# EleutherAI/DALLE-mtf

Measured on AMD Instinct MI355X. Metric: train tokens/sec (text+image) per node, dalle_example, higher is better.
Workload: dtype bf16

## Files before the change

### dalle-mtf_amd/csrc/gemm.hip

```cpp
#include "common.h"
#include <string.h>
#include <type_traits>

static int g_opt_nt4 = 1;
static int g_opt_nt8 = 1;
int g_opt_reserve_cus = 0;
int g_opt_attn_fwd = 1;
int g_opt_attn_bwd = 1;
int g_opt_attn_xcd = 8;
static int g_opt_tn8 = 0;
static int g_opt_tn8_max_tiles = 16;
static int g_opt_nt8_min_k = 2048;
static int g_opt_skinny = 1;
static int g_opt_tn_wide = 1;
static int g_opt_tn_tail = 1;
static int g_opt_cstream = 1;
static int g_opt_cstream_min_mb = 256;
static int g_opt_cstream_nt_min_mb = 1024;
static int g_opt_res16 = 1;
static int g_opt_ntr = 1;
static int g_opt_nt8p = 1;
static int g_opt_relu_bits = 1;
static int g_opt_nt8p_max_k = 1024;
static int g_opt_nt4_lds = 49152;
unsigned long long* g_dbg_buf = nullptr;
extern "C" int dmi_set_debug_buffer(void* p) { g_dbg_buf = (unsigned long long*)p; return 0; }
extern "C" int dmi_get_option(const char* name) {
  if (!strcmp(name, "nt4")) return g_opt_nt4;
  if (!strcmp(name, "nt8")) return g_opt_nt8;
  if (!strcmp(name, "tn_tail")) return g_opt_tn_tail;
  if (!strcmp(name, "tn_wide")) return g_opt_tn_wide;
  if (!strcmp(name, "nt4_lds")) return g_opt_nt4_lds;
  if (!strcmp(name, "nt8p")) return g_opt_nt8p;
  if (!strcmp(name, "ntr")) return g_opt_ntr;
  if (!strcmp(name, "cstream")) return g_opt_cstream;
  if (!strcmp(name, "cstream_min_mb")) return g_opt_cstream_min_mb;
  if (!strcmp(name, "cstream_nt_min_mb")) return g_opt_cstream_nt_min_mb;
  if (!strcmp(name, "nt8p_max_k")) return g_opt_nt8p_max_k;
  if (!strcmp(name, "relu_bits")) return g_opt_relu_bits;
  if (!strcmp(name, "res16")) return g_opt_res16;
  if (!strcmp(name, "skinny")) return g_opt_skinny;
  if (!strcmp(name, "nt8_min_k")) return g_opt_nt8_min_k;
  if (!strcmp(name, "tn8")) return g_opt_tn8;
  if (!strcmp(name, "tn8_max_tiles")) return g_opt_tn8_max_tiles;
  if (!strcmp(name, "attn_xcd")) return g_opt_attn_xcd;
  if (!strcmp(name, "attn_fwd")) return g_opt_attn_fwd;
  if (!strcmp(name, "attn_bwd")) return g_opt_attn_bwd;
  if (!strcmp(name, "reserve_cus")) return g_opt_reserve_cus;
  return -1;
}
extern "C" int dmi_set_option(const char* name, int value) {
  if (!strcmp(name, "nt4")) { g_opt_nt4 = value; return 0; }
  if (!strcmp(name, "nt8")) { g_opt_nt8 = value; return 0; }
  if (!strcmp(name, "tn_tail")) { g_opt_tn_tail = value; return 0; }
  if (!strcmp(name, "tn_wide")) { g_opt_tn_wide = value; return 0; }
  if (!strcmp(name, "nt4_lds")) { if (value < 49152 || value > 163840) return -1; g_opt_nt4_lds = value; return 0; }
  if (!strcmp(name, "nt8p")) { g_opt_nt8p = value; return 0; }
  if (!strcmp(name, "ntr")) { g_opt_ntr = value; return 0; }
  if (!strcmp(name, "cstream")) { g_opt_cstream = value; return 0; }
  if (!strcmp(name, "cstream_min_mb")) { g_opt_cstream_min_mb = value; return 0; }
  if (!strcmp(name, "cstream_nt_min_mb")) { g_opt_cstream_nt_min_mb = value; return 0; }
  if (!strcmp(name, "nt8p_max_k")) { g_opt_nt8p_max_k = value; return 0; }
  if (!strcmp(name, "relu_bits")) { g_opt_relu_bits = value; return 0; }
  if (!strcmp(name, "res16")) { g_opt_res16 = value; return 0; }
  if (!strcmp(name, "skinny")) { g_opt_skinny = value; return 0; }
  if (!strcmp(name, "nt8_min_k")) { g_opt_nt8_min_k = value; return 0; }
  if (!strcmp(name, "tn8")) { g_opt_tn8 = value; return 0; }
  if (!strcmp(name, "tn8_max_tiles")) { g_opt_tn8_max_tiles = value; return 0; }
  if (!strcmp(name, "attn_xcd")) { g_opt_attn_xcd = value; return 0; }
  if (!strcmp(name, "attn_fwd")) { g_opt_attn_fwd = value; return 0; }
  if (!strcmp(name, "attn_bwd")) { g_opt_attn_bwd = value; return 0; }
  if (!strcmp(name, "reserve_cus")) { if (value < 0) return -1; g_opt_reserve_cus = value; return 0; }
  return -1;
}

#define BM 128
#define BN 128
#define BK 64
#ifndef GROUP_M
#define GROUP_M 8
#endif

struct GemmArgs {
  const bf16_t* A;
  const bf16_t* B;
  void* C;
  const bf16_t* bias;
  const bf16_t* residual;
  const bf16_t* relu_src;
  unsigned short* relu_bits;
  const float* rowscale;
// ... 888 lines not shown
      const u32x2 graw = *(const u32x2*)(a.ln_gamma + n), braw = *(const u32x2*)(a.ln_beta + n);
      const float g0 = __uint_as_float(graw[0] << 16), g1 = __uint_as_float(graw[0] & 0xffff0000u);
      const float g2 = __uint_as_float(graw[1] << 16), g3 = __uint_as_float(graw[1] & 0xffff0000u);
      const float b0 = __uint_as_float(braw[0] << 16), b1 = __uint_as_float(braw[0] & 0xffff0000u);
      const float b2 = __uint_as_float(braw[1] << 16), b3 = __uint_as_float(braw[1] & 0xffff0000u);
#pragma unroll
      for (int t = 0; t < RT; ++t) {
        P[t][jj][0] = pack2bf(acc[t][j][0] * rs[t] * g0 + b0, acc[t][j][1] * rs[t] * g1 + b1);
        P[t][jj][1] = pack2bf(acc[t][j][2] * rs[t] * g2 + b2, acc[t][j][3] * rs[t] * g3 + b3);
      }
    }
#pragma unroll
    for (int t = 0; t < RT; ++t) {
      const int m = m0 + wm * (RM / 2) + 16 * t + c16;
#pragma unroll
      for (int d = 0; d < 2; ++d) { swap16(P[t][0][d], P[t][1][d]); swap16(P[t][2][d], P[t][3][d]); }
      if (m < a.M) {
        bf16_t* yp = a.ln_y + (int64_t)m * a.ln_ldy + ncolw + 64 * h + pcol;
        *(u32x4*)yp = u32x4{P[t][0][0], P[t][0][1], P[t][1][0], P[t][1][1]};
        *(u32x4*)(yp + 32) = u32x4{P[t][2][0], P[t][2][1], P[t][3][0], P[t][3][1]};
      }
    }
  }
}

__device__ __forceinline__ float dpp_row_sum16(float v) {
  v += __builtin_bit_cast(float, __builtin_amdgcn_update_dpp(0, __builtin_bit_cast(int, v), 0xB1, 0xf, 0xf, false));
  v += __builtin_bit_cast(float, __builtin_amdgcn_update_dpp(0, __builtin_bit_cast(int, v), 0x4E, 0xf, 0xf, false));
  v += __builtin_bit_cast(float, __builtin_amdgcn_update_dpp(0, __builtin_bit_cast(int, v), 0x141, 0xf, 0xf, false));
  v += __builtin_bit_cast(float, __builtin_amdgcn_update_dpp(0, __builtin_bit_cast(int, v), 0x140, 0xf, 0xf, false));
  return v;
}
template <int RT>
__device__ __forceinline__ void epilogue_lnbwd(const GemmArgs& a, f32x4 (&acc)[RT][8], char* smem, int lane, int wm, int wn, int m0) {
  constexpr int RM = 32 * RT;
  const int c16 = lane & 15, g16 = lane >> 4;
  float* red = (float*)smem;
  const int ncolw = wn * 128;
  const int pcol = 8 * (((g16 & 1) << 1) | (g16 >> 1));
  const float invn = 1.0f / 512.0f;
  const int nbytes = (int)(((int64_t)(a.M - m0) * 512) * 2);
  const __amdgpu_buffer_rsrc_t rx = __builtin_amdgcn_make_buffer_rsrc((void*)(a.ln_x + (int64_t)m0 * 512), 0, nbytes, 0x00020000);
  const __amdgpu_buffer_rsrc_t rr = __builtin_amdgcn_make_buffer_rsrc((void*)((a.residual ? a.residual : a.ln_x) + (int64_t)m0 * 512), 0,
                                                                       a.residual ? nbytes : 0, 0x00020000);
  const __amdgpu_buffer_rsrc_t ry = __builtin_amdgcn_make_buffer_rsrc((void*)(a.ln_y + (int64_t)m0 * 512), 0, nbytes, 0x00020000);
  const __amdgpu_buffer_rsrc_t rmu = __builtin_amdgcn_make_buffer_rsrc((void*)(a.ln_mean + m0), 0, (a.M - m0) * 4, 0x00020000);
  const __amdgpu_buffer_rsrc_t rrs = __builtin_amdgcn_make_buffer_rsrc((void*)(a.ln_rstd + m0), 0, (a.M - m0) * 4, 0x00020000);
  const int r0 = wm * (RM / 2) + c16;
  float* prow = a.ln_part + (int64_t)(blockIdx.x * 2 + wm) * 1024;
  auto lo = [](unsigned w) { return __uint_as_float(w << 16); };
  auto hi = [](unsigned w) { return __uint_as_float(w & 0xffff0000u); };
  unsigned dyp[RT][8][2], xp[RT][8][2];
  const int vst = (r0 * 512 + ncolw + pcol) * 2;
  auto ld16 = [&](const __amdgpu_buffer_rsrc_t rsrc, int voff, int imm) {
    return __builtin_bit_cast(u32x4, __builtin_amdgcn_raw_buffer_load_b128(rsrc, voff, imm, 0));
  };
  auto ldmu = [&](int t) { return __builtin_bit_cast(float, __builtin_amdgcn_raw_buffer_load_b32(rmu, r0 * 4 + 64 * t, 0, 0)); };
  auto ldrs = [&](int t) { return __builtin_bit_cast(float, __builtin_amdgcn_raw_buffer_load_b32(rrs, r0 * 4 + 64 * t, 0, 0)); };
  const bf16_t* gp = a.ln_gamma + ncolw + 4 * g16;
#pragma unroll
  for (int t = 0; t < RT; ++t)
#pragma unroll
    for (int h = 0; h < 2; ++h) {
      const u32x4 l0 = ld16(rx, vst + 16384 * t + 128 * h, 0), l1 = ld16(rx, vst + 16384 * t + 128 * h + 64, 0);
      xp[t][4 * h + 0][0] = l0[0]; xp[t][4 * h + 0][1] = l0[1]; xp[t][4 * h + 1][0] = l0[2]; xp[t][4 * h + 1][1] = l0[3];
      xp[t][4 * h + 2][0] = l1[0]; xp[t][4 * h + 2][1] = l1[1]; xp[t][4 * h + 3][0] = l1[2]; xp[t][4 * h + 3][1] = l1[3];
    }
#pragma unroll
  for (int t = 0; t < RT; ++t)
#pragma unroll
    for (int j = 0; j < 8; ++j) {
      dyp[t][j][0] = pack2bf(acc[t][j][0], acc[t][j][1]); dyp[t][j][1] = pack2bf(acc[t][j][2], acc[t][j][3]);
      asm volatile("" : "+v"(dyp[t][j][0]), "+v"(dyp[t][j][1]));
    }
#pragma unroll
  for (int t = 0; t < RT; ++t)
#pragma unroll
    for (int h = 0; h < 2; ++h)
#pragma unroll
      for (int dd = 0; dd < 2; ++dd) { swap16(xp[t][4 * h][dd], xp[t][4 * h + 1][dd]); swap16(xp[t][4 * h + 2][dd], xp[t][4 * h + 3][dd]); }
  auto opaque = [&]() {
#pragma unroll
    for (int t = 0; t < RT; ++t)
#pragma unroll
      for (int j = 0; j < 8; ++j) asm volatile("" : "+v"(dyp[t][j][0]), "+v"(dyp[t][j][1]), "+v"(xp[t][j][0]), "+v"(xp[t][j][1]));
  };
  opaque();
  float s1[RT], s2[RT];
  {
    unsigned gmp[8][2];
#pragma unroll
    for (int j = 0; j < 8; ++j) {
      const u32x2 graw = *(const u32x2*)(gp + 16 * j);
      gmp[j][0] = graw[0]; gmp[j][1] = graw[1];
    }
#pragma unroll
    for (int t = 0; t < RT; ++t) {
      const float mu = ldmu(t), rs = ldrs(t);
      float a1 = 0.f, a2 = 0.f;
#pragma unroll
      for (int j = 0; j < 8; ++j) {
        const float xv[4] = {lo(xp[t][j][0]), hi(xp[t][j][0]), lo(xp[t][j][1]), hi(xp[t][j][1])};
        const float dy[4] = {lo(dyp[t][j][0]), hi(dyp[t][j][0]), lo(dyp[t][j][1]), hi(dyp[t][j][1])};
        const float gm[4] = {lo(gmp[j][0]), hi(gmp[j][0]), lo(gmp[j][1]), hi(gmp[j][1])};
#pragma unroll
        for (int e = 0; e < 4; ++e) {
          const float xh = (xv[e] - mu) * rs;
          const float gy = dy[e] * gm[e];
          a1 += gy;
          a2 += gy * xh;
        }
      }
      s1[t] = a1; s2[t] = a2;
      __builtin_amdgcn_sched_barrier(0);
    }
  }
#pragma unroll
  for (int t = 0; t < RT; ++t) {
    s1[t] += __shfl_xor(s1[t], 16, 64); s1[t] += __shfl_xor(s1[t], 32, 64);
    s2[t] += __shfl_xor(s2[t], 16, 64); s2[t] += __shfl_xor(s2[t], 32, 64);
    if (g16 == 0) {
      float* q = red + ((r0 + 16 * t) * 4 + wn) * 2;
      q[0] = s1[t]; q[1] = s2[t];
    }
  }
  __syncthreads();
  opaque();
  {
    float mu[RT], rs[RT];
#pragma unroll
    for (int t = 0; t < RT; ++t) { mu[t] = ldmu(t); rs[t] = ldrs(t); }
#pragma unroll
    for (int j = 0; j < 8; ++j) {
      float ag[4] = {0.f, 0.f, 0.f, 0.f}, ab[4] = {0.f, 0.f, 0.f, 0.f};
#pragma unroll
      for (int t = 0; t < RT; ++t) {
        const float xv[4] = {lo(xp[t][j][0]), hi(xp[t][j][0]), lo(xp[t][j][1]), hi(xp[t][j][1])};
        const float dy[4] = {lo(dyp[t][j][0]), hi(dyp[t][j][0]), lo(dyp[t][j][1]), hi(dyp[t][j][1])};
#pragma unroll
        for (int e = 0; e < 4; ++e) {
          ab[e] += dy[e];
          ag[e] += dy[e] * ((xv[e] - mu[t]) * rs[t]);
        }
      }
      f32x4 pg, pb;
#pragma unroll
      for (int e = 0; e < 4; ++e) { pg[e] = dpp_row_sum16(ag[e]); pb[e] = dpp_row_sum16(ab[e]); }
      if (c16 == 0) {
        const int n = ncolw + 16 * j + 4 * g16;
        *(f32x4*)(prow + n) = pg;
        *(f32x4*)(prow + 512 + n) = pb;
      }
      __builtin_amdgcn_sched_barrier(0);
    }
  }
  opaque();
#pragma unroll
  for (int t = 0; t < RT; ++t) {
    const f32x4 q0 = *(const f32x4*)(red + (r0 + 16 * t) * 8);
    const f32x4 q1 = *(const f32x4*)(red + (r0 + 16 * t) * 8 + 4);
    const float m1 = ((q0[0] + q0[2]) + (q1[0] + q1[2])) * invn;
    const float m2 = ((q0[1] + q0[3]) + (q1[1] + q1[3])) * invn;
    const float mu = ldmu(t), rs = ldrs(t);
#pragma unroll
    for (int h = 0; h < 2; ++h) {
      const u32x4 l0 = ld16(rr, vst + 16384 * t + 128 * h, 0), l1 = ld16(rr, vst + 16384 * t + 128 * h + 64, 0);
      unsigned R[4][2] = {{l0[0], l0[1]}, {l0[2], l0[3]}, {l1[0], l1[1]}, {l1[2], l1[3]}};
#pragma unroll
      for (int dd = 0; dd < 2; ++dd) { swap16(R[0][dd], R[1][dd]); swap16(R[2][dd], R[3][dd]); }
      unsigned P[4][2];
#pragma unroll
      for (int jj = 0; jj < 4; ++jj) {
        const int j = 4 * h + jj;
        const u32x2 graw = *(const u32x2*)(gp + 16 * j);
        const float xv[4] = {lo(xp[t][j][0]), hi(xp[t][j][0]), lo(xp[t][j][1]), hi(xp[t][j][1])};
        const float rv[4] = {lo(R[jj][0]), hi(R[jj][0]), lo(R[jj][1]), hi(R[jj][1])};
        const float gm[4] = {lo(graw[0]), hi(graw[0]), lo(graw[1]), hi(graw[1])};
        const float dy[4] = {lo(dyp[t][j][0]), hi(dyp[t][j][0]), lo(dyp[t][j][1]), hi(dyp[t][j][1])};
        float o[4];
#pragma unroll
        for (int e = 0; e < 4; ++e) {
          const float xh = (xv[e] - mu) * rs;
          o[e] = rs * (dy[e] * gm[e] - m1 - xh * m2) + rv[e];
        }
        P[jj][0] = pack2bf(o[0], o[1]);
        P[jj][1] = pack2bf(o[2], o[3]);
      }
#pragma unroll
      for (int dd = 0; dd < 2; ++dd) { swap16(P[0][dd], P[1][dd]); swap16(P[2][dd], P[3][dd]); }
      __builtin_amdgcn_raw_buffer_store_b128(u32x4{P[0][0], P[0][1], P[1][0], P[1][1]}, ry, vst + 16384 * t + 128 * h, 0, 0);
      __builtin_amdgcn_raw_buffer_store_b128(u32x4{P[2][0], P[2][1], P[3][0], P[3][1]}, ry, vst + 16384 * t + 128 * h + 64, 0, 0);
      __builtin_amdgcn_sched_barrier(0);
    }
  }
}

template <int FLAGS, int RT, int LN = 0>
__global__ __launch_bounds__(512, 2) void gemm_ntr_kernel(GemmArgs a) {
  extern __shared__ __attribute__((aligned(16))) char smem[];
  constexpr int RM = 32 * RT;
  constexpr int ABYTES = RM * 64;
  constexpr int BUF = ABYTES + 32768;
  constexpr int NPA = RM / 16;
  constexpr int NP = NPA + 32;
  constexpr int PW = (NP + 7) / 8;
  const int tid = threadIdx.x, lane = tid & 63;
  const int wid = __builtin_amdgcn_readfirstlane(tid >> 6);
  const int wm = wid >> 2, wn = wid & 3;
  const int m0 = blockIdx.x * RM;
  int ns = a.K / 32;

  const int c16 = lane & 15, g16 = lane >> 4;
  int offa = lds4_off(wm * (RM / 2) + c16, g16);
  int offb = ABYTES + lds4_off(wn * 128 + c16, g16);
  __amdgpu_buffer_rsrc_t ra = __builtin_amdgcn_make_buffer_rsrc((void*)(a.A + (int64_t)m0 * a.lda), 0,
                                                                 (int)(((int64_t)(a.M - 1 - m0) * a.lda + a.K) * 2), 0x00020000);
  __amdgpu_buffer_rsrc_t rb = __builtin_amdgcn_make_buffer_rsrc((void*)a.B, 0, (int)(((int64_t)(a.N - 1) * a.ldb + a.K) * 2), 0x00020000);
  int vo[PW];
  auto set_offsets = [&](int lda_, int ldb_, int ln) {
#pragma unroll
    for (int q = 0; q < PW; ++q) {
      const int p = wid + 8 * q;
      const bool isa = p < NPA;
      const int row = 16 * (isa ? p : p - NPA) + (ln >> 2), pc = ln & 3;
      vo[q] = (row * (isa ? lda_ : ldb_) + 8 * (pc ^ lds4_swz(row))) * 2;
    }
  };
  set_offsets(a.lda, a.ldb, lane);
  auto piece = [&](int buf, int q, int soff) {
    const int p = wid + 8 * q;
    if (p >= NP) return;
    char* dst = smem + buf * BUF + (p < NPA ? p * 1024 : ABYTES + (p - NPA) * 1024);
    if (p < NPA) glds16(ra, dst, vo[q], soff);
    else glds16(rb, dst, vo[q], soff);
  };

  f32x4 acc[RT][8];
#pragma unroll
  for (int i = 0; i < RT; ++i)
#pragma unroll
    for (int j = 0; j < 8; ++j) acc[i][j] = f32x4{0.f, 0.f, 0.f, 0.f};

  auto compute = [&](int buf, int nbuf, int soff) {
    const char* cur = smem + buf * BUF;
    bf16x8 fb[8], fa[RT];
#pragma unroll
    for (int j = 0; j < 8; ++j) fb[j] = *(const bf16x8*)(cur + offb + j * 1024);
    fa[0] = *(const bf16x8*)(cur + offa);
    if (RT > 1) fa[1] = *(const bf16x8*)(cur + offa + 1024);
    MFMA_PRIO(1);
#pragma unroll
    for (int i = 0; i < RT; ++i) {
      if (i + 2 < RT) fa[i + 2] = *(const bf16x8*)(cur + offa + (i + 2) * 1024);
#pragma unroll
      for (int j = 0; j < 8; ++j)
        acc[i][j] = __builtin_amdgcn_mfma_f32_16x16x32_bf16(fb[j], fa[i], acc[i][j], 0, 0, 0);
#pragma unroll
      for (int q = 2 * i; q < 2 * i + 2; ++q)
        if (q < PW) piece(nbuf, q, soff);
      __builtin_amdgcn_sched_barrier(0);
    }
    MFMA_PRIO(0);
  };

  auto mainloop = [&]() {
#pragma unroll
    for (int q = 0; q < PW; ++q) piece(0, q, 0);
#pragma unroll
    for (int q = 0; q < PW; ++q) piece(1, q, ns > 1 ? 64 : 0);
    asm volatile("s_waitcnt vmcnt(0)" ::: "memory");
    __syncthreads();
    for (int s = 0; s < ns; s += 3) {
#pragma unroll
      for (int u = 0; u < 3; ++u) {
        if (s + u < ns) {
          const int q = s + u + 2;
          compute(u, (u + 2) % 3, (q < ns ? q : 0) * 64);
          asm volatile("s_waitcnt vmcnt(%0)" ::"n"(PW - 1) : "memory");
          __builtin_amdgcn_s_barrier();
        }
      }
    }
    asm volatile("s_waitcnt vmcnt(0)" ::: "memory");
  };
  mainloop();
  if constexpr (LN == 3) {
    __syncthreads();
    {
      int lane_e = (int)__builtin_amdgcn_mbcnt_hi(~0u, __builtin_amdgcn_mbcnt_lo(~0u, 0u));
      asm volatile("" : "+v"(lane_e));
      epilogue_lnbwd<RT>(a, acc, smem, lane_e, wm, wn, m0);
    }
    asm volatile("s_waitcnt vmcnt(0)" ::: "memory");
    __syncthreads();
    ra = __builtin_amdgcn_make_buffer_rsrc((void*)(a.ln_y + (int64_t)m0 * a.ln_ldy), 0, (int)(((int64_t)(a.M - 1 - m0) * a.ln_ldy + a.N) * 2), 0x00020000);
    rb = __builtin_amdgcn_make_buffer_rsrc((void*)a.B2, 0, (int)(((int64_t)(a.N - 1) * a.ldb2 + a.N) * 2), 0x00020000);
    int lane2 = (int)__builtin_amdgcn_mbcnt_hi(~0u, __builtin_amdgcn_mbcnt_lo(~0u, 0u));
    asm volatile("" : "+v"(lane2));
    offa = lds4_off(wm * (RM / 2) + (lane2 & 15), lane2 >> 4);
    offb = ABYTES + lds4_off(wn * 128 + (lane2 & 15), lane2 >> 4);
    set_offsets(a.ln_ldy, a.ldb2, lane2);
    ns = a.N / 32;
#pragma unroll
    for (int i = 0; i < RT; ++i)
#pragma unroll
      for (int j = 0; j < 8; ++j) acc[i][j] = f32x4{0.f, 0.f, 0.f, 0.f};
    mainloop();
    GemmArgs b2 = a;
    b2.C = a.C2; b2.ldc = a.N; b2.cpol = 0;
    f32x4 lo[RT][4], hi[RT][4];
#pragma unroll
    for (int i = 0; i < RT; ++i)
#pragma unroll
      for (int j = 0; j < 4; ++j) { lo[i][j] = acc[i][j]; hi[i][j] = acc[i][j + 4]; }
    epilogue_regs<0, RT>(b2, lo, lane2, m0 + wm * (RM / 2), wn * 128);
    epilogue_regs<0, RT>(b2, hi, lane2, m0 + wm * (RM / 2), wn * 128 + 64);
  } else if constexpr (LN != 0) {
    __syncthreads();
    if constexpr (LN == 1) epilogue_ln<RT>(a, acc, smem, lane, wm, wn, m0);
    else {
      int lane_e = lane;
      asm volatile("" : "+v"(lane_e));
      epilogue_lnbwd<RT>(a, acc, smem, lane_e, wm, wn, m0);
    }
  } else {
    f32x4 lo[RT][4], hi[RT][4];
#pragma unroll
    for (int i = 0; i < RT; ++i)
#pragma unroll
      for (int j = 0; j < 4; ++j) { lo[i][j] = acc[i][j]; hi[i][j] = acc[i][j + 4]; }
    epilogue_regs<FLAGS, RT>(a, lo, lane, m0 + wm * (RM / 2), wn * 128);
    epilogue_regs<FLAGS, RT>(a, hi, lane, m0 + wm * (RM / 2), wn * 128 + 64);
  }
}

__global__ __launch_bounds__(256) void reduce_slabs_kernel(const float* __restrict__ slabs, float* __restrict__ out,
                                                           int nsplit, int64_t n4, int64_t stride4) {
  for (int64_t i = (int64_t)blockIdx.x * 256 + threadIdx.x; i < n4; i += (int64_t)gridDim.x * 256) {
    f32x4 acc = ((const f32x4*)slabs)[i];
    for (int s = 1; s < nsplit; ++s) {
      const f32x4 v = ((const f32x4*)slabs)[s * stride4 + i];
      acc[0] += v[0]; acc[1] += v[1]; acc[2] += v[2]; acc[3] += v[3];
    }
    ((f32x4*)out)[i] = acc;
  }
}

#define SK_WAVES 8
template <int FLAGS>
__global__ __launch_bounds__(64 * SK_WAVES) void gemm_nt_skinny_kernel(const GemmArgs a) {
  __shared__ f32x4 red[SK_WAVES][2][64];
  const int lane = threadIdx.x & 63, wid = threadIdx.x >> 6;
  const int c = lane & 15, g = lane >> 4;
  const int n0 = blockIdx.x * 16;
  const int r0 = c < a.M ? c : a.M - 1, r1 = 16 + c < a.M ? 16 + c : a.M - 1;
  const bf16_t* pa0 = a.A + (int64_t)r0 * a.lda + 16 * g;
// ... 136 lines not shown
static int num_cus() {
  static int n = 0;
  if (!n) {
    int dev = 0;
    hipDeviceProp_t prop;
    if (hipGetDevice(&dev) == hipSuccess && hipGetDeviceProperties(&prop, dev) == hipSuccess) n = prop.multiProcessorCount;
    if (n < 8) n = 256;
  }
  return n;
}

static int persistent_grid() {
  int n = (num_cus() - g_opt_reserve_cus) & ~7;
  return n < 8 ? 8 : n;
}

static bool nt8p_can(const GemmArgs& a) {
  return a.k_per_split == a.K && a.K % 128 == 0 && (int64_t)a.M * a.lda < (1 << 30) && (int64_t)a.N * a.ldb < (1 << 30);
}
static bool nt8p_auto(int M, int N, int K) {
  return K <= g_opt_nt8p_max_k && ((M + BM8 - 1) / BM8) * ((N + BN8 - 1) / BN8) >= 2 * num_cus();
}
template <int FLAGS>
static int launch_nt8p(const GemmArgs& a, hipStream_t st) {
  static bool attr8p = false;
  if (!attr8p) { (void)hipFuncSetAttribute((const void*)gemm_nt8p_kernel<FLAGS>, hipFuncAttributeMaxDynamicSharedMemorySize, 131072); attr8p = true; }
  GemmArgs b = a;
  b.tiles_m = (a.M + BM8 - 1) / BM8; b.tiles_n = (a.N + BN8 - 1) / BN8;
  gemm_nt8p_kernel<FLAGS><<<dim3(persistent_grid()), dim3(512), 131072, st>>>(b);
  DMI_CHECK_LAUNCH("gemm_nt8p");
  return DMI_OK;
}

template <int FLAGS>
static int launch_nt(const GemmArgs& a, int nsplit, hipStream_t st) {
  const dim3 grid(a.tiles_m * a.tiles_n, nsplit), blk(256);
  if constexpr (FLAGS == 0 || FLAGS == DMI_GEMM_BIAS || FLAGS == (DMI_GEMM_BIAS | DMI_GEMM_RELU) || FLAGS == (DMI_GEMM_BIAS | DMI_GEMM_RESIDUAL)) {
    if (g_opt_skinny && a.M <= 32 && nsplit == 1 && a.N % 16 == 0) {
      gemm_nt_skinny_kernel<FLAGS><<<dim3(a.N / 16), dim3(64 * SK_WAVES), 0, st>>>(a);
      DMI_CHECK_LAUNCH("gemm_nt_skinny");
      return DMI_OK;
    }
  }
  if constexpr (epi_regs_ok<FLAGS> && !(FLAGS & GEMM_SOFTMAX)) {
    if (g_opt_ntr && a.N == 512 && nsplit == 1 && a.k_per_split == a.K && a.K % 32 == 0 && (int64_t)a.N * a.ldb < (1 << 30) &&
        (g_opt_ntr == 2 || (a.M >= 160 * (num_cus() / 2) && a.K <= 4096 && g_opt_reserve_cus == 0))) {
      constexpr int RT = 5;
      constexpr int LDSB = 3 * (32 * RT * 64 + 32768);
      static bool attrr = false;
      if (!attrr) { (void)hipFuncSetAttribute((const void*)gemm_ntr_kernel<FLAGS, RT>, hipFuncAttributeMaxDynamicSharedMemorySize, LDSB); attrr = true; }
      GemmArgs b = a;
      b.pf = g_opt_res16 ? 2 : 0;
      gemm_ntr_kernel<FLAGS, RT><<<dim3((a.M + 32 * RT - 1) / (32 * RT)), dim3(512), LDSB, st>>>(b);
      DMI_CHECK_LAUNCH("gemm_ntr");
      return DMI_OK;
    }
  }
  if constexpr (epi_regs_ok<FLAGS>) {
    const bool can = nsplit == 1 && nt8p_can(a);
    const bool auto_ok = nt8p_auto(a.M, a.N, a.K);
    if (can && ((g_opt_nt8p == 1 && auto_ok) || g_opt_nt8p == 2 || (g_opt_nt8p == 3 && (FLAGS & GEMM_SOFTMAX) && auto_ok)))
      return launch_nt8p<FLAGS>(a, st);
  }
  {
    const int t8m = (a.M + BM8 - 1) / BM8, t8n = (a.N + BN8 - 1) / BN8;
    const bool auto8 = g_opt_nt8 == 1 && a.k_per_split >= g_opt_nt8_min_k && (t8m * t8n * nsplit) % 256 == 0;
    if (auto8 || g_opt_nt8 == 2) {
      static bool attr8 = false;
      if (!attr8) { (void)hipFuncSetAttribute((const void*)gemm_nt8_kernel<FLAGS>, hipFuncAttributeMaxDynamicSharedMemorySize, 131072); attr8 = true; }
      GemmArgs b = a;
      b.tiles_m = t8m; b.tiles_n = t8n;
      gemm_nt8_kernel<FLAGS><<<dim3(t8m * t8n, nsplit), dim3(512), 131072, st>>>(b);
      DMI_CHECK_LAUNCH("gemm_nt8");
      return DMI_OK;
    }
  }
  if constexpr (!(FLAGS & DMI_GEMM_OUT_F32)) {
    const int tiles4 = ((a.M + BM4 - 1) / BM4) * a.tiles_n;
    if (g_opt_nt4 && nsplit == 1 && a.k_per_split == a.K && ((tiles4 >= 1536 && a.K <= 1024) || g_opt_nt4 == 2)) {
      static int attr4 = 0;
      if (attr4 != g_opt_nt4_lds) { (void)hipFuncSetAttribute((const void*)gemm_nt4_kernel<FLAGS>, hipFuncAttributeMaxDynamicSharedMemorySize, g_opt_nt4_lds); attr4 = g_opt_nt4_lds; }
      GemmArgs b = a;
      b.tiles_m = (a.M + BM4 - 1) / BM4;
      gemm_nt4_kernel<FLAGS><<<dim3(tiles4), blk, g_opt_nt4_lds, st>>>(b);
      DMI_CHECK_LAUNCH("gemm_nt4");
      return DMI_OK;
// ... 83 lines not shown
extern "C" int dmi_gemm_nt_mask_bits(const uint16_t* A, int lda, const uint16_t* Bt, int ldb, uint16_t* C, int ldc, int M, int N, int K,
                                     const void* bits, void* stream) {
  int rc = check_nt(A, lda, Bt, ldb, C, ldc, M, N, K);
  if (rc) return rc;
  GemmArgs a;
  fill_nt_args(a, A, lda, Bt, ldb, C, ldc, M, N, K);
  a.relu_bits = (unsigned short*)bits; a.dbg = g_dbg_buf;
  if ((rc = check_bits("gemm_nt_mask_bits", a, bits))) return rc;
  return launch_nt8p<GEMM_MASK_BITS>(a, (hipStream_t)stream);
}

extern "C" int dmi_gemm_nt_ln_auto(int M, int N, int K) {
  if (M <= 0 || N != 512 || K <= 0 || K % BK != 0) return 0;
  if ((int64_t)N * K >= (1 << 30) || (int64_t)M * K >= ((int64_t)1 << 31) || (int64_t)M * N * 2 >= ((int64_t)1 << 31)) return 0;
  return g_opt_reserve_cus == 0 ? 1 : 0;
}

extern "C" int dmi_gemm_nt_ln(const uint16_t* A, int lda, const uint16_t* Bt, int ldb, uint16_t* C, int ldc, int M, int N, int K,
                              const uint16_t* bias, const uint16_t* residual, const uint16_t* gamma, const uint16_t* beta, float eps,
                              uint16_t* Y, int ldy, float* mean, float* rstd, void* stream) {
  int rc = check_nt(A, lda, Bt, ldb, C, ldc, M, N, K);
  if (rc) return rc;
  DMI_REQUIRE(gamma && beta && Y && mean && rstd, "gemm_nt_ln: null pointer");
  DMI_REQUIRE((((uintptr_t)gamma | (uintptr_t)beta | (uintptr_t)Y | (uintptr_t)bias | (uintptr_t)residual) & 15) == 0 && ldy % 8 == 0 && ldy >= N,
              "gemm_nt_ln: operands must be 16-byte aligned");
  if (N != 512 || (int64_t)N * ldb >= (1 << 30) || (int64_t)M * lda >= ((int64_t)1 << 31)) {
    dmi_set_error("gemm_nt_ln: the fused form needs N = 512 (one block owns whole rows); got N=%d", N);
    return DMI_ERR_UNSUPPORTED;
  }
  GemmArgs a;
  fill_nt_args(a, A, lda, Bt, ldb, C, ldc, M, N, K);
  a.bias = bias; a.residual = residual;
  a.ln_gamma = gamma; a.ln_beta = beta; a.ln_y = Y; a.ln_ldy = ldy; a.ln_mean = mean; a.ln_rstd = rstd; a.ln_eps = eps;
  constexpr int RT = 5;
  constexpr int LDSB = 3 * (32 * RT * 64 + 32768);
  static bool attr = false;
  if (!attr) { (void)hipFuncSetAttribute((const void*)gemm_ntr_kernel<0, RT, 1>, hipFuncAttributeMaxDynamicSharedMemorySize, LDSB); attr = true; }
  gemm_ntr_kernel<0, RT, 1><<<dim3((M + 32 * RT - 1) / (32 * RT)), dim3(512), LDSB, (hipStream_t)stream>>>(a);
  DMI_CHECK_LAUNCH("gemm_nt_ln");
  return DMI_OK;
}

extern "C" int dmi_gemm_nt_lnbwd_parts(int M) { return 2 * ((M + 159) / 160); }
extern "C" int dmi_gemm_nt_lnbwd(const uint16_t* A, int lda, const uint16_t* Bt, int ldb, int M, int N, int K, const uint16_t* x,
                                 const uint16_t* gamma, const float* mean, const float* rstd, const uint16_t* dres, uint16_t* dx,
                                 float* part, const uint16_t* B2, int ldb2, uint16_t* C2, void* stream) {
  int rc = check_nt(A, lda, Bt, ldb, dx, N, M, N, K);
  if (rc) return rc;
  DMI_REQUIRE(x && gamma && mean && rstd && part, "gemm_nt_lnbwd: null pointer");
  DMI_REQUIRE((((uintptr_t)x | (uintptr_t)gamma | (uintptr_t)dres | (uintptr_t)part) & 15) == 0, "gemm_nt_lnbwd: operands must be 16-byte aligned");
  if (N != 512 || (int64_t)N * ldb >= (1 << 30) || (int64_t)M * lda >= ((int64_t)1 << 31) || (int64_t)M * N * 2 >= ((int64_t)1 << 31)) {
    dmi_set_error("gemm_nt_lnbwd: the fused form needs N = 512 (one block owns whole rows) and operands below 2 GiB; got M=%d N=%d", M, N);
    return DMI_ERR_UNSUPPORTED;
  }
  GemmArgs a;
  fill_nt_args(a, A, lda, Bt, ldb, dx, N, M, N, K);
  a.residual = dres; a.ln_x = x; a.ln_gamma = gamma; a.ln_mean = (float*)mean; a.ln_rstd = (float*)rstd; a.ln_y = dx; a.ln_ldy = N; a.ln_part = part;
  constexpr int RT = 5;
  constexpr int LDSB = 3 * (32 * RT * 64 + 32768);
  if (B2 || C2) {
    DMI_REQUIRE(B2 && C2 && ldb2 >= N && ldb2 % 8 == 0 && (((uintptr_t)B2 | (uintptr_t)C2) & 15) == 0 && (const void*)C2 != (const void*)dx,
                "gemm_nt_lnbwd: bad chained product (B2 / ldb2 / C2)");
    a.B2 = B2; a.ldb2 = ldb2; a.C2 = C2;
    static bool attr3 = false;
    if (!attr3) { (void)hipFuncSetAttribute((const void*)gemm_ntr_kernel<0, RT, 3>, hipFuncAttributeMaxDynamicSharedMemorySize, LDSB); attr3 = true; }
    gemm_ntr_kernel<0, RT, 3><<<dim3((M + 32 * RT - 1) / (32 * RT)), dim3(512), LDSB, (hipStream_t)stream>>>(a);
    DMI_CHECK_LAUNCH("gemm_nt_lnbwd (chained)");
    return DMI_OK;
  }
  static bool attr = false;
  if (!attr) { (void)hipFuncSetAttribute((const void*)gemm_ntr_kernel<0, RT, 2>, hipFuncAttributeMaxDynamicSharedMemorySize, LDSB); attr = true; }
  gemm_ntr_kernel<0, RT, 2><<<dim3((M + 32 * RT - 1) / (32 * RT)), dim3(512), LDSB, (hipStream_t)stream>>>(a);
  DMI_CHECK_LAUNCH("gemm_nt_lnbwd");
  return DMI_OK;
}

extern "C" int dmi_ln_gemm_nt(const uint16_t* X, int ldx, const uint16_t* gamma, const uint16_t* beta, float eps, const uint16_t* Bt, int ldb,
                              uint16_t* C, int ldc, int M, int N, int K, int flags, const uint16_t* bias, void* stream) {
  int rc = check_nt(X, ldx, Bt, ldb, C, ldc, M, N, K);
  if (rc) return rc;
  DMI_REQUIRE(gamma && beta, "ln_gemm_nt: null LayerNorm parameters");
  DMI_REQUIRE((((uintptr_t)gamma | (uintptr_t)beta) & 15) == 0, "ln_gemm_nt: gamma / beta must be 16-byte aligned");
  DMI_REQUIRE(!(flags & DMI_GEMM_BIAS) || bias, "ln_gemm_nt: bias flag without pointer");
  if (M > 32 || N % 16 != 0 || K > 64 * SK_WAVES * SKLN_MAXSTEPS) {
    dmi_set_error("ln_gemm_nt: only the decode-step shapes (M <= 32, N %% 16 == 0, K <= %d); got M=%d N=%d K=%d", 64 * SK_WAVES * SKLN_MAXSTEPS, M, N, K);
    return DMI_ERR_UNSUPPORTED;
  }
  GemmArgs a;
  fill_nt_args(a, X, ldx, Bt, ldb, C, ldc, M, N, K);
  a.bias = bias;
  const dim3 grid(N / 16), blk(64 * SK_WAVES);
  hipStream_t st = (hipStream_t)stream;
  switch (flags) {
    case 0: gemm_ln_nt_skinny_kernel<0><<<grid, blk, 0, st>>>(a, gamma, beta, eps); break;
    case DMI_GEMM_BIAS: gemm_ln_nt_skinny_kernel<DMI_GEMM_BIAS><<<grid, blk, 0, st>>>(a, gamma, beta, eps); break;
    case DMI_GEMM_BIAS | DMI_GEMM_RELU: gemm_ln_nt_skinny_kernel<DMI_GEMM_BIAS | DMI_GEMM_RELU><<<grid, blk, 0, st>>>(a, gamma, beta, eps); break;
    default:
      dmi_set_error("ln_gemm_nt: unsupported flag combination %d", flags);
      return DMI_ERR_UNSUPPORTED;
  }
  DMI_CHECK_LAUNCH("ln_gemm_nt");
  return DMI_OK;
}

extern "C" int dmi_gemm_nt_softmax(const uint16_t* A, int lda, const uint16_t* Bt, int ldb, const uint16_t* bias,
// ... 1371 lines not shown
```

Before: 2.852 million.

## Add split-workgroup variant of row-owning GEMM and prefetch LN-backward epilogue loads

Adds a HALF template variant of the row-owning NT GEMM kernel. It uses 256 threads per workgroup, each owning half the rows of a tile, with a two-stage LDS pipeline, and is compiled only under NTR_TWO_WORKGROUPS behind an ntr_overlap option that defaults to off. The LayerNorm-backward epilogue now loads mean/rstd and gamma before its loops and software-pipelines the residual-gradient loads one step ahead, so memory latency overlaps the arithmetic. Launch code is unified into a launch_ntr helper. The half variant is meant to let two smaller workgroups overlap epilogue and mainloop on a CU, at the cost of duplicated B-tile loads and shallower pipelining. The epilogue prefetch raises register pressure.

```diff
diff --git a/dalle-mtf_amd/csrc/gemm.hip b/dalle-mtf_amd/csrc/gemm.hip
--- a/dalle-mtf_amd/csrc/gemm.hip
+++ b/dalle-mtf_amd/csrc/gemm.hip
@@ -19,6 +19,11 @@
 static int g_opt_cstream_nt_min_mb = 1024;
 static int g_opt_res16 = 1;
 static int g_opt_ntr = 1;
+#ifdef NTR_TWO_WORKGROUPS
+static int g_opt_ntr_overlap = 0;
+#else
+static constexpr int g_opt_ntr_overlap = 0;
+#endif
 static int g_opt_nt8p = 1;
 static int g_opt_relu_bits = 1;
 static int g_opt_nt8p_max_k = 1024;
@@ -33,6 +38,9 @@
   if (!strcmp(name, "nt4_lds")) return g_opt_nt4_lds;
   if (!strcmp(name, "nt8p")) return g_opt_nt8p;
   if (!strcmp(name, "ntr")) return g_opt_ntr;
+#ifdef NTR_TWO_WORKGROUPS
+  if (!strcmp(name, "ntr_overlap")) return g_opt_ntr_overlap;
+#endif
   if (!strcmp(name, "cstream")) return g_opt_cstream;
   if (!strcmp(name, "cstream_min_mb")) return g_opt_cstream_min_mb;
   if (!strcmp(name, "cstream_nt_min_mb")) return g_opt_cstream_nt_min_mb;
@@ -57,6 +65,9 @@
   if (!strcmp(name, "nt4_lds")) { if (value < 49152 || value > 163840) return -1; g_opt_nt4_lds = value; return 0; }
   if (!strcmp(name, "nt8p")) { g_opt_nt8p = value; return 0; }
   if (!strcmp(name, "ntr")) { g_opt_ntr = value; return 0; }
+#ifdef NTR_TWO_WORKGROUPS
+  if (!strcmp(name, "ntr_overlap")) { if (value < 0 || value > 2) return -1; g_opt_ntr_overlap = value; return 0; }
+#endif
   if (!strcmp(name, "cstream")) { g_opt_cstream = value; return 0; }
   if (!strcmp(name, "cstream_min_mb")) { g_opt_cstream_min_mb = value; return 0; }
   if (!strcmp(name, "cstream_nt_min_mb")) { g_opt_cstream_nt_min_mb = value; return 0; }
@@ -1011,7 +1022,7 @@
   return v;
 }
 template <int RT>
-__device__ __forceinline__ void epilogue_lnbwd(const GemmArgs& a, f32x4 (&acc)[RT][8], char* smem, int lane, int wm, int wn, int m0) {
+__device__ __forceinline__ void epilogue_lnbwd(const GemmArgs& a, f32x4 (&acc)[RT][8], char* smem, int lane, int wm, int wn, int m0, int tile) {
   constexpr int RM = 32 * RT;
   const int c16 = lane & 15, g16 = lane >> 4;
   float* red = (float*)smem;
@@ -1026,7 +1037,7 @@
   const __amdgpu_buffer_rsrc_t rmu = __builtin_amdgcn_make_buffer_rsrc((void*)(a.ln_mean + m0), 0, (a.M - m0) * 4, 0x00020000);
   const __amdgpu_buffer_rsrc_t rrs = __builtin_amdgcn_make_buffer_rsrc((void*)(a.ln_rstd + m0), 0, (a.M - m0) * 4, 0x00020000);
   const int r0 = wm * (RM / 2) + c16;
-  float* prow = a.ln_part + (int64_t)(blockIdx.x * 2 + wm) * 1024;
+  float* prow = a.ln_part + (int64_t)(tile * 2 + wm) * 1024;
   auto lo = [](unsigned w) { return __uint_as_float(w << 16); };
   auto hi = [](unsigned w) { return __uint_as_float(w & 0xffff0000u); };
   unsigned dyp[RT][8][2], xp[RT][8][2];
@@ -1073,9 +1084,12 @@
       const u32x2 graw = *(const u32x2*)(gp + 16 * j);
       gmp[j][0] = graw[0]; gmp[j][1] = graw[1];
     }
+    float mu1[RT], rs1[RT];
+#pragma unroll
+    for (int t = 0; t < RT; ++t) { mu1[t] = ldmu(t); rs1[t] = ldrs(t); }
 #pragma unroll
     for (int t = 0; t < RT; ++t) {
-      const float mu = ldmu(t), rs = ldrs(t);
+      const float mu = mu1[t], rs = rs1[t];
       float a1 = 0.f, a2 = 0.f;
 #pragma unroll
       for (int j = 0; j < 8; ++j) {
@@ -1134,16 +1148,29 @@
     }
   }
   opaque();
+  int vst2 = vst;
+  asm volatile("" : "+v"(vst2));
+  float mu2[RT], rs2[RT];
+  u32x2 gm2[8];
+#pragma unroll
+  for (int j = 0; j < 8; ++j) gm2[j] = *(const u32x2*)(gp + 16 * j);
+#pragma unroll
+  for (int t = 0; t < RT; ++t) { mu2[t] = ldmu(t); rs2[t] = ldrs(t); }
+  u32x4 dn0 = ld16(rr, vst2, 0), dn1 = ld16(rr, vst2 + 64, 0);
 #pragma unroll
   for (int t = 0; t < RT; ++t) {
     const f32x4 q0 = *(const f32x4*)(red + (r0 + 16 * t) * 8);
     const f32x4 q1 = *(const f32x4*)(red + (r0 + 16 * t) * 8 + 4);
     const float m1 = ((q0[0] + q0[2]) + (q1[0] + q1[2])) * invn;
     const float m2 = ((q0[1] + q0[3]) + (q1[1] + q1[3])) * invn;
-    const float mu = ldmu(t), rs = ldrs(t);
+    const float mu = mu2[t], rs = rs2[t];
 #pragma unroll
     for (int h = 0; h < 2; ++h) {
-      const u32x4 l0 = ld16(rr, vst + 16384 * t + 128 * h, 0), l1 = ld16(rr, vst + 16384 * t + 128 * h + 64, 0);
+      const u32x4 l0 = dn0, l1 = dn1;
+      if (2 * t + h + 1 < 2 * RT) {
+        const int nt = (2 * t + h + 1) / 2, nh = (2 * t + h + 1) % 2;
+        dn0 = ld16(rr, vst2 + 16384 * nt + 128 * nh, 0); dn1 = ld16(rr, vst2 + 16384 * nt + 128 * nh + 64, 0);
+      }
       unsigned R[4][2] = {{l0[0], l0[1]}, {l0[2], l0[3]}, {l1[0], l1[1]}, {l1[2], l1[3]}};
 #pragma unroll
       for (int dd = 0; dd < 2; ++dd) { swap16(R[0][dd], R[1][dd]); swap16(R[2][dd], R[3][dd]); }
@@ -1151,7 +1178,7 @@
 #pragma unroll
       for (int jj = 0; jj < 4; ++jj) {
         const int j = 4 * h + jj;
-        const u32x2 graw = *(const u32x2*)(gp + 16 * j);
+        const u32x2 graw = gm2[j];
         const float xv[4] = {lo(xp[t][j][0]), hi(xp[t][j][0]), lo(xp[t][j][1]), hi(xp[t][j][1])};
         const float rv[4] = {lo(R[jj][0]), hi(R[jj][0]), lo(R[jj][1]), hi(R[jj][1])};
         const float gm[4] = {lo(graw[0]), hi(graw[0]), lo(graw[1]), hi(graw[1])};
@@ -1167,51 +1194,71 @@
       }
 #pragma unroll
       for (int dd = 0; dd < 2; ++dd) { swap16(P[0][dd], P[1][dd]); swap16(P[2][dd], P[3][dd]); }
-      __builtin_amdgcn_raw_buffer_store_b128(u32x4{P[0][0], P[0][1], P[1][0], P[1][1]}, ry, vst + 16384 * t + 128 * h, 0, 0);
-      __builtin_amdgcn_raw_buffer_store_b128(u32x4{P[2][0], P[2][1], P[3][0], P[3][1]}, ry, vst + 16384 * t + 128 * h + 64, 0, 0);
+      __builtin_amdgcn_raw_buffer_store_b128(u32x4{P[0][0], P[0][1], P[1][0], P[1][1]}, ry, vst2 + 16384 * t + 128 * h, 0, 0);
+      __builtin_amdgcn_raw_buffer_store_b128(u32x4{P[2][0], P[2][1], P[3][0], P[3][1]}, ry, vst2 + 16384 * t + 128 * h + 64, 0, 0);
       __builtin_amdgcn_sched_barrier(0);
     }
   }
 }
 
-template <int FLAGS, int RT, int LN = 0>
-__global__ __launch_bounds__(512, 2) void gemm_ntr_kernel(GemmArgs a) {
+template <int FLAGS, int RT, int LN = 0, int HALF = 0>
+__global__ __launch_bounds__(HALF ? 256 : 512, 2) void gemm_ntr_kernel(GemmArgs a) {
   extern __shared__ __attribute__((aligned(16))) char smem[];
+  constexpr int NW = HALF ? 4 : 8;
+  constexpr int NST = HALF ? 2 : 3;
   constexpr int RM = 32 * RT;
-  constexpr int ABYTES = RM * 64;
+  constexpr int RMB = HALF ? RM / 2 : RM;
+  constexpr int ABYTES = RMB * 64;
   constexpr int BUF = ABYTES + 32768;
-  constexpr int NPA = RM / 16;
+  constexpr int NPA = RMB / 16;
   constexpr int NP = NPA + 32;
-  constexpr int PW = (NP + 7) / 8;
+  constexpr int PW = (NP + NW - 1) / NW;
+  constexpr int PPG = HALF ? 4 : 2;
+  static_assert(PW <= PPG * RT, "every piece needs a slot behind an MFMA group");
   const int tid = threadIdx.x, lane = tid & 63;
   const int wid = __builtin_amdgcn_readfirstlane(tid >> 6);
-  const int wm = wid >> 2, wn = wid & 3;
-  const int m0 = blockIdx.x * RM;
+  const int wm = HALF ? (int)(blockIdx.x & 1) : wid >> 2, wn = wid & 3;
+  const int tile = HALF ? (int)(blockIdx.x >> 1) : (int)blockIdx.x;
+  const int m0 = tile * RM;
+  const int arow = HALF ? wm * (RM / 2) : 0;
+  const int wrow = HALF ? 0 : wm * (RM / 2);
   int ns = a.K / 32;
 
   const int c16 = lane & 15, g16 = lane >> 4;
-  int offa = lds4_off(wm * (RM / 2) + c16, g16);
+  int offa = lds4_off(wrow + c16, g16);
   int offb = ABYTES + lds4_off(wn * 128 + c16, g16);
   __amdgpu_buffer_rsrc_t ra = __builtin_amdgcn_make_buffer_rsrc((void*)(a.A + (int64_t)m0 * a.lda), 0,
                                                                  (int)(((int64_t)(a.M - 1 - m0) * a.lda + a.K) * 2), 0x00020000);
   __amdgpu_buffer_rsrc_t rb = __builtin_amdgcn_make_buffer_rsrc((void*)a.B, 0, (int)(((int64_t)(a.N - 1) * a.ldb + a.K) * 2), 0x00020000);
-  int vo[PW];
+  constexpr int QV = HALF ? (NPA + NW - 1) / NW : PW;
+  int vo[QV], vob = 0, ldbs = a.ldb;
   auto set_offsets = [&](int lda_, int ldb_, int ln) {
 #pragma unroll
-    for (int q = 0; q < PW; ++q) {
-      const int p = wid + 8 * q;
+    for (int q = 0; q < QV; ++q) {
+      const int p = wid + NW * q;
       const bool isa = p < NPA;
       const int row = 16 * (isa ? p : p - NPA) + (ln >> 2), pc = ln & 3;
-      vo[q] = (row * (isa ? lda_ : ldb_) + 8 * (pc ^ lds4_swz(row))) * 2;
-    }
+      vo[q] = ((row + (isa ? arow : 0)) * (isa ? lda_ : ldb_) + 8 * (pc ^ lds4_swz(row))) * 2;
+    }
+    vob = ((ln >> 2) * ldb_ + 8 * ((ln & 3) ^ lds4_swz(ln >> 2))) * 2;
+    ldbs = ldb_;
   };
   set_offsets(a.lda, a.ldb, lane);
+  int sbq = 0, ldq = 0;
+  auto bterms = [&](int soff) {
+    sbq = soff + 32 * (wid + NW * QV - NPA) * ldbs; ldq = 32 * NW * ldbs;
+    asm volatile("" : "+s"(sbq), "+s"(ldq));
+  };
   auto piece = [&](int buf, int q, int soff) {
-    const int p = wid + 8 * q;
+    const int p = wid + NW * q;
     if (p >= NP) return;
     char* dst = smem + buf * BUF + (p < NPA ? p * 1024 : ABYTES + (p - NPA) * 1024);
-    if (p < NPA) glds16(ra, dst, vo[q], soff);
-    else glds16(rb, dst, vo[q], soff);
+    if (q < QV) {
+      if (p < NPA) glds16(ra, dst, vo[q < QV ? q : 0], soff);
+      else glds16(rb, dst, vo[q < QV ? q : 0], soff);
+    } else {
+      glds16(rb, dst, vob, sbq + (q - QV) * ldq);
+    }
   };
 
   f32x4 acc[RT][8];
@@ -1220,8 +1267,9 @@
 #pragma unroll
     for (int j = 0; j < 8; ++j) acc[i][j] = f32x4{0.f, 0.f, 0.f, 0.f};
 
-  auto compute = [&](int buf, int nbuf, int soff) {
+  auto compute = [&](int buf, int nbuf, int soff, bool ld) {
     const char* cur = smem + buf * BUF;
+    if (QV < PW) bterms(soff);
     bf16x8 fb[8], fa[RT];
 #pragma unroll
     for (int j = 0; j < 8; ++j) fb[j] = *(const bf16x8*)(cur + offb + j * 1024);
@@ -1235,28 +1283,47 @@
       for (int j = 0; j < 8; ++j)
         acc[i][j] = __builtin_amdgcn_mfma_f32_16x16x32_bf16(fb[j], fa[i], acc[i][j], 0, 0, 0);
 #pragma unroll
-      for (int q = 2 * i; q < 2 * i + 2; ++q)
-        if (q < PW) piece(nbuf, q, soff);
+      for (int q = PPG * i; q < PPG * i + PPG; ++q)
+        if (q < PW && ld) piece(nbuf, q, soff);
       __builtin_amdgcn_sched_barrier(0);
     }
     MFMA_PRIO(0);
   };
 
   auto mainloop = [&]() {
-#pragma unroll
-    for (int q = 0; q < PW; ++q) piece(0, q, 0);
-#pragma unroll
-    for (int q = 0; q < PW; ++q) piece(1, q, ns > 1 ? 64 : 0);
-    asm volatile("s_waitcnt vmcnt(0)" ::: "memory");
-    __syncthreads();
-    for (int s = 0; s < ns; s += 3) {
-#pragma unroll
-      for (int u = 0; u < 3; ++u) {
-        if (s + u < ns) {
-          const int q = s + u + 2;
-          compute(u, (u + 2) % 3, (q < ns ? q : 0) * 64);
-          asm volatile("s_waitcnt vmcnt(%0)" ::"n"(PW - 1) : "memory");
-          __builtin_amdgcn_s_barrier();
+    if constexpr (NST == 3) {
+#pragma unroll
+      for (int q = 0; q < PW; ++q) piece(0, q, 0);
+#pragma unroll
+      for (int q = 0; q < PW; ++q) piece(1, q, ns > 1 ? 64 : 0);
+      asm volatile("s_waitcnt vmcnt(0)" ::: "memory");
+      __syncthreads();
+      for (int s = 0; s < ns; s += 3) {
+#pragma unroll
+        for (int u = 0; u < 3; ++u) {
+          if (s + u < ns) {
+            const int q = s + u + 2;
+            compute(u, (u + 2) % 3, (q < ns ? q : 0) * 64, true);
+            asm volatile("s_waitcnt vmcnt(%0)" ::"n"(PW - 1) : "memory");
+            __builtin_amdgcn_s_barrier();
+          }
+        }
+      }
+    } else {
+      bterms(0);
+#pragma unroll
+      for (int q = 0; q < PW; ++q) piece(0, q, 0);
+      asm volatile("s_waitcnt vmcnt(0)" ::: "memory");
+      __syncthreads();
+      for (int s = 0; s < ns; s += 2) {
+#pragma unroll
+        for (int u = 0; u < 2; ++u) {
+          if (s + u < ns) {
+            const int q = s + u + 1;
+            compute(u, u ^ 1, q * 64, q < ns);
+            asm volatile("s_waitcnt vmcnt(0)" ::: "memory");
+            __builtin_amdgcn_s_barrier();
+          }
         }
       }
     }
@@ -1268,7 +1335,7 @@
     {
       int lane_e = (int)__builtin_amdgcn_mbcnt_hi(~0u, __builtin_amdgcn_mbcnt_lo(~0u, 0u));
       asm volatile("" : "+v"(lane_e));
-      epilogue_lnbwd<RT>(a, acc, smem, lane_e, wm, wn, m0);
+      epilogue_lnbwd<RT>(a, acc, smem, lane_e, wm, wn, m0, tile);
     }
     asm volatile("s_waitcnt vmcnt(0)" ::: "memory");
     __syncthreads();
@@ -1276,7 +1343,7 @@
     rb = __builtin_amdgcn_make_buffer_rsrc((void*)a.B2, 0, (int)(((int64_t)(a.N - 1) * a.ldb2 + a.N) * 2), 0x00020000);
     int lane2 = (int)__builtin_amdgcn_mbcnt_hi(~0u, __builtin_amdgcn_mbcnt_lo(~0u, 0u));
     asm volatile("" : "+v"(lane2));
-    offa = lds4_off(wm * (RM / 2) + (lane2 & 15), lane2 >> 4);
+    offa = lds4_off(wrow + (lane2 & 15), lane2 >> 4);
     offb = ABYTES + lds4_off(wn * 128 + (lane2 & 15), lane2 >> 4);
     set_offsets(a.ln_ldy, a.ldb2, lane2);
     ns = a.N / 32;
@@ -1300,7 +1367,7 @@
     else {
       int lane_e = lane;
       asm volatile("" : "+v"(lane_e));
-      epilogue_lnbwd<RT>(a, acc, smem, lane_e, wm, wn, m0);
+      epilogue_lnbwd<RT>(a, acc, smem, lane_e, wm, wn, m0, tile);
     }
   } else {
     f32x4 lo[RT][4], hi[RT][4];
@@ -1503,6 +1570,28 @@
   return DMI_OK;
 }
 
+template <int FLAGS, int LN>
+static void launch_ntr(const GemmArgs& a, bool half, hipStream_t st) {
+  constexpr int RT = 5;
+  const int tiles = (a.M + 32 * RT - 1) / (32 * RT);
+#ifdef NTR_TWO_WORKGROUPS
+  if (half) {
+    constexpr int LDSB = 2 * (16 * RT * 64 + 32768);
+    static bool attr = false;
+    if (!attr) { (void)hipFuncSetAttribute((const void*)gemm_ntr_kernel<FLAGS, RT, LN, 1>, hipFuncAttributeMaxDynamicSharedMemorySize, LDSB); attr = true; }
+    gemm_ntr_kernel<FLAGS, RT, LN, 1><<<dim3(2 * tiles), dim3(256), LDSB, st>>>(a);
+    return;
+  }
+#endif
+  (void)half;
+  {
+    constexpr int LDSB = 3 * (32 * RT * 64 + 32768);
+    static bool attr = false;
+    if (!attr) { (void)hipFuncSetAttribute((const void*)gemm_ntr_kernel<FLAGS, RT, LN>, hipFuncAttributeMaxDynamicSharedMemorySize, LDSB); attr = true; }
+    gemm_ntr_kernel<FLAGS, RT, LN><<<dim3(tiles), dim3(512), LDSB, st>>>(a);
+  }
+}
+
 template <int FLAGS>
 static int launch_nt(const GemmArgs& a, int nsplit, hipStream_t st) {
   const dim3 grid(a.tiles_m * a.tiles_n, nsplit), blk(256);
@@ -1516,13 +1605,9 @@
   if constexpr (epi_regs_ok<FLAGS> && !(FLAGS & GEMM_SOFTMAX)) {
     if (g_opt_ntr && a.N == 512 && nsplit == 1 && a.k_per_split == a.K && a.K % 32 == 0 && (int64_t)a.N * a.ldb < (1 << 30) &&
         (g_opt_ntr == 2 || (a.M >= 160 * (num_cus() / 2) && a.K <= 4096 && g_opt_reserve_cus == 0))) {
-      constexpr int RT = 5;
-      constexpr int LDSB = 3 * (32 * RT * 64 + 32768);
-      static bool attrr = false;
-      if (!attrr) { (void)hipFuncSetAttribute((const void*)gemm_ntr_kernel<FLAGS, RT>, hipFuncAttributeMaxDynamicSharedMemorySize, LDSB); attrr = true; }
       GemmArgs b = a;
       b.pf = g_opt_res16 ? 2 : 0;
-      gemm_ntr_kernel<FLAGS, RT><<<dim3((a.M + 32 * RT - 1) / (32 * RT)), dim3(512), LDSB, st>>>(b);
+      launch_ntr<FLAGS, 0>(b, g_opt_ntr_overlap == 2, st);
       DMI_CHECK_LAUNCH("gemm_ntr");
       return DMI_OK;
     }
@@ -1672,11 +1757,7 @@
   fill_nt_args(a, A, lda, Bt, ldb, C, ldc, M, N, K);
   a.bias = bias; a.residual = residual;
   a.ln_gamma = gamma; a.ln_beta = beta; a.ln_y = Y; a.ln_ldy = ldy; a.ln_mean = mean; a.ln_rstd = rstd; a.ln_eps = eps;
-  constexpr int RT = 5;
-  constexpr int LDSB = 3 * (32 * RT * 64 + 32768);
-  static bool attr = false;
-  if (!attr) { (void)hipFuncSetAttribute((const void*)gemm_ntr_kernel<0, RT, 1>, hipFuncAttributeMaxDynamicSharedMemorySize, LDSB); attr = true; }
-  gemm_ntr_kernel<0, RT, 1><<<dim3((M + 32 * RT - 1) / (32 * RT)), dim3(512), LDSB, (hipStream_t)stream>>>(a);
+  launch_ntr<0, 1>(a, g_opt_ntr_overlap != 0, (hipStream_t)stream);
   DMI_CHECK_LAUNCH("gemm_nt_ln");
   return DMI_OK;
 }
@@ -1696,21 +1777,15 @@
   GemmArgs a;
   fill_nt_args(a, A, lda, Bt, ldb, dx, N, M, N, K);
   a.residual = dres; a.ln_x = x; a.ln_gamma = gamma; a.ln_mean = (float*)mean; a.ln_rstd = (float*)rstd; a.ln_y = dx; a.ln_ldy = N; a.ln_part = part;
-  constexpr int RT = 5;
-  constexpr int LDSB = 3 * (32 * RT * 64 + 32768);
   if (B2 || C2) {
     DMI_REQUIRE(B2 && C2 && ldb2 >= N && ldb2 % 8 == 0 && (((uintptr_t)B2 | (uintptr_t)C2) & 15) == 0 && (const void*)C2 != (const void*)dx,
                 "gemm_nt_lnbwd: bad chained product (B2 / ldb2 / C2)");
     a.B2 = B2; a.ldb2 = ldb2; a.C2 = C2;
-    static bool attr3 = false;
-    if (!attr3) { (void)hipFuncSetAttribute((const void*)gemm_ntr_kernel<0, RT, 3>, hipFuncAttributeMaxDynamicSharedMemorySize, LDSB); attr3 = true; }
-    gemm_ntr_kernel<0, RT, 3><<<dim3((M + 32 * RT - 1) / (32 * RT)), dim3(512), LDSB, (hipStream_t)stream>>>(a);
+    launch_ntr<0, 3>(a, g_opt_ntr_overlap != 0, (hipStream_t)stream);
     DMI_CHECK_LAUNCH("gemm_nt_lnbwd (chained)");
     return DMI_OK;
   }
-  static bool attr = false;
-  if (!attr) { (void)hipFuncSetAttribute((const void*)gemm_ntr_kernel<0, RT, 2>, hipFuncAttributeMaxDynamicSharedMemorySize, LDSB); attr = true; }
-  gemm_ntr_kernel<0, RT, 2><<<dim3((M + 32 * RT - 1) / (32 * RT)), dim3(512), LDSB, (hipStream_t)stream>>>(a);
+  launch_ntr<0, 2>(a, g_opt_ntr_overlap != 0, (hipStream_t)stream);
   DMI_CHECK_LAUNCH("gemm_nt_lnbwd");
   return DMI_OK;
 }
```

After: 2.860 million, median of 6. About the same (+0.3%).
